# dluvizon/scene-aware-3d-multi-human

Hardware: AMD Instinct MI355X
Metric: optimizer iterations/sec (N humans x T frames) (higher is better)
Workload: dtype f32 (the two dense LBS contractions as split-16-bit MFMA operands -- three products of (hi, lo) fp16 / bf16 terms, fp32 accumulate; everything else plain fp32)

## Files before the change

### include/mhmocap_hip.h

```cpp
#ifndef MHMOCAP_HIP_H
#define MHMOCAP_HIP_H

#include <stddef.h>
#include <stdint.h>

#ifdef __cplusplus
extern "C" {
#endif

#define MH_NUM_JOINTS 24
#define MH_NUM_BETAS 10
#define MH_NUM_POSE_BASIS 207
#define MH_NUM_KP 17
#define MH_FEAT_STRIDE 224

typedef enum mh_status {
  MH_OK = 0,
  MH_ERR_INVALID = -1,
  MH_ERR_HIP = -2,
  MH_ERR_NO_DEVICE = -3,
  MH_ERR_UNSUPPORTED = -4
} mh_status;

typedef struct mh_model mh_model;
// ... 27 lines not shown
};
int mh_profile_enable(int on);
int mh_profile_read(int which, float* ms);
int mh_device_count(void);

int mh_stream_create(void** out_stream);
int mh_stream_destroy(void* stream);
int mh_streams_share_queue(void* stream_a, void* stream_b, float spin_us, int* shared);
int mh_stream_spin(void* stream, float spin_us);

int mh_model_create(mh_model** out, const mh_model_host* host);
int mh_model_destroy(mh_model* m);
const int32_t* mh_model_faces(const mh_model* m);

size_t mh_lbs_workspace_bytes(int B);
int mh_lbs_forward(const mh_model* m, int B, int NB, const float* betas ,
                   const float* poses , const float* xscale ,
                   const float* transl , float* verts ,
                   float* vposed , float* posed_joints ,
                   void* ws, void* stream);

int mh_lbs_forward_ex(const mh_model* m, int B, int NB, const float* betas, const float* poses ,
                      const float* rotmats , const float* xscale, const float* transl, float* verts,
                      float* vposed , float* posed_joints , void* ws, void* stream);
int mh_lbs_forward_rotmats(const mh_model* m, int B, int NB, const float* betas, const float* rotmats ,
                           const float* xscale, const float* transl, float* verts, float* posed_joints ,
                           void* ws, void* stream);

typedef struct mh_fwd_proj {
  float s, w1, h1;
  float ra, rk, thr;
  float slack_ndc, slack_y;
  float thr_soft;
  float* ndc;
  const float* rowb;
  int32_t* bbox;
  int32_t* bbox_prev;
  unsigned long long* lowkey;
  unsigned long long* lowkey_prev;
  int32_t* moved;
  float* clear;
  unsigned long long clear_n;
} mh_fwd_proj;
int mh_lbs_forward_proj(const mh_model* m, int B, int NB, const float* betas, const float* poses,
                        const float* xscale, const float* transl, float* verts, float* vposed ,
                        const mh_fwd_proj* proj, void* ws, void* stream);
int mh_lowest_resolve(const float* verts , int B, int V, unsigned long long* lowkey ,
                      int32_t* low_idx , float* low_xyz , void* stream);

int mh_lbs_set_mode(int split16);
int mh_lbs_get_mode(void);
int mh_lbs_set_forward_pipeline(int on);
int mh_lbs_get_forward_pipeline(void);

int mh_joints_regress(const mh_model* m, int which, int B, const float* verts ,
                      const float* corr , int root_relative_to,
                      float* joints , void* stream);

size_t mh_keypoint_workspace_bytes(const mh_model* m, int B);
int mh_keypoint_terms(const mh_model* m, int B, const float* transl , const float* K_host,
                      const float* Kd_host , const float* joint_w_host ,
                      const float* pose2d , float thr, float img_w, float img_h, float coef,
                      float* kp, float* uv, float* gkp, float* loss, const void* ws, void* ws2 ,
                      void* kp_ws, void* stream);
int mh_lbs_backward_kp(const mh_model* m, int B, int NB, const float* betas, const float* poses,
                       const float* vposed, const float* gverts, float* gposes, float* gtransl,
                       float* gbetas, float* gxscale, void* ws, void* ws2, void* stream);
typedef struct mh_raster_fin mh_raster_fin;
int mh_lbs_backward_kp_fin(const mh_model* m, int B, int NB, const float* betas, const float* poses,
                       const float* vposed, const float* gverts, float* gposes, float* gtransl,
                       float* gbetas, float* gxscale, void* ws, void* ws2, const mh_raster_fin* fin, void* stream);

int mh_lbs_backward_person_partials(const mh_model* m, int B, void* ws2, float** gbeta_b, float** gxs_b);
int mh_lbs_person_reduce(const mh_model* m, int B, int NB, void* ws2, float* gbetas, float* gxscale, void* stream);

size_t mh_lbs_backward_workspace_bytes(int B);
int mh_lbs_backward(const mh_model* m, int B, int NB, const float* betas, const float* poses,
                    const float* xscale, const float* transl, const float* vposed,
                    const float* gverts, const float* gjoints, float* gposes, float* gtransl,
                    float* gbetas, float* gxscale, void* ws, void* ws2, void* stream);
int mh_lbs_backward_ex(const mh_model* m, int B, int NB, const float* betas, const float* poses, const float* rotmats,
                       const float* vposed, const float* gverts, const float* gjoints, const float* gposed,
                       float* gposes, float* grotmats, float* gtransl, float* gbetas, float* gxscale,
                       void* ws, void* ws2, void* stream);
int mh_joints_regress_backward(const mh_model* m, int which, int B, const float* gjoints , int root_relative_to,
                               float* gverts, float* gcorr, void* stream);

int mh_project_joints_loss(int B, const float* joints , const float* K_host,
                           const float* Kd_host, const float* pose2d, float thr, int mode,
                           float img_w, float img_h, float coef, float* uv, float* gjoints,
                           float* loss, void* stream);

int mh_project_joints_loss_w(int B, const float* joints, const float* K_host, const float* Kd_host,
                             const float* joint_w_host, const float* pose2d, float thr, int mode, float img_w,
                             float img_h, float coef, float* uv, float* gjoints, float* loss, void* stream);

int mh_warmup_project(int B, int NB, const float* local_joints , const float* xscale,
                      const float* transl , const float* K_host, const float* Kd_host,
                      const float* pose2d, float thr, float coef, float* gtransl, float* loss,
                      void* stream);

int mh_warmup_project_w(int B, int NB, const float* local_joints, const float* xscale, const float* transl,
                        const float* K_host, const float* Kd_host, const float* joint_w_host, const float* pose2d,
                        float thr, float coef, float* gtransl, float* loss, void* stream);

int mh_rmsprop_step(float* params, const float* grads, float* square_avg, float* momentum_buf,
// ... 224 lines not shown
```

### scene-aware-3d-multi-human_amd/csrc/mh_lbs.hip

```cpp
#include <algorithm>
#include <mutex>
#include <unordered_map>

#include "mh_common.h"
#include "mh_raster_p.h"
#include "mh_experiment.h"

#define MFMA32(a, b, c) __builtin_amdgcn_mfma_f32_32x32x2f32((a), (b), (c), 0, 0, 0)


struct PoseFwdP {
  int B, NB, G;
  const float* betas;
  const float* poses;
  const float* rotmats;
  const float* xscale;
  const float* Jt;
  const float* JS;
  float* featT;
  uint16_t* F16;
  float* A;
  float* scale;
  float* posed;
  mh_tree tree;
  int* bbox;
  int* bbox_prev;
  unsigned long long* lowkey;
  unsigned long long* lowkey_prev;
  int* moved;
  float* clear;
  unsigned long long clear_n;
};

__device__ __forceinline__ void mh_joint_rest(const float* Jt, const float* JS, const float* beta, int j, float J[3]) {
#pragma unroll
  for (int c = 0; c < 3; ++c) {
    float a = Jt[j * 3 + c];
#pragma unroll
    for (int l = 0; l < MH_NUM_BETAS; ++l) a = fmaf(JS[(j * 3 + c) * MH_NUM_BETAS + l], beta[l], a);
    J[c] = a;
  }
}

__device__ __forceinline__ void mh_compose(const float* Gp, const float R[9], const float rel[3], float G[12]) {
#pragma unroll
  for (int r = 0; r < 3; ++r) {
#pragma unroll
    for (int c = 0; c < 3; ++c)
      G[r * 4 + c] = fmaf(Gp[r * 4 + 2], R[6 + c], fmaf(Gp[r * 4 + 1], R[3 + c], Gp[r * 4 + 0] * R[c]));
    G[r * 4 + 3] = fmaf(Gp[r * 4 + 2], rel[2], fmaf(Gp[r * 4 + 1], rel[1], Gp[r * 4 + 0] * rel[0])) + Gp[r * 4 + 3];
  }
}

__global__ __launch_bounds__(256) void k_pose_fwd(PoseFwdP p) {
  __shared__ float sG[8][MH_NJ][12];
  __shared__ float sJ[8][MH_NJ][3];
  if (p.clear)
    for (size_t i = (size_t)blockIdx.x * 256 + threadIdx.x; i < p.clear_n; i += (size_t)gridDim.x * 256) p.clear[i] = 0.f;
  const int bl = threadIdx.x >> 5, j = threadIdx.x & 31;
  const int b = blockIdx.x * 8 + bl;
  const bool valid = b < p.B, act = j < MH_NJ;
  float beta[MH_NUM_BETAS];
#pragma unroll
  for (int l = 0; l < MH_NUM_BETAS; ++l) beta[l] = valid ? p.betas[(size_t)(b % p.NB) * MH_NUM_BETAS + l] : 0.f;
  float R[9] = {1, 0, 0, 0, 1, 0, 0, 0, 1}, J[3] = {0, 0, 0};
  if (valid && act) {
    mh_joint_rest(p.Jt, p.JS, beta, j, J);
    if (p.rotmats) {
#pragma unroll
      for (int e = 0; e < 9; ++e) R[e] = p.rotmats[((size_t)b * MH_NJ + j) * 9 + e];
    } else if (j < 22) {
      float r[3] = {p.poses[(size_t)b * 72 + 3 * j], p.poses[(size_t)b * 72 + 3 * j + 1], p.poses[(size_t)b * 72 + 3 * j + 2]};
      mh_rodrigues(r, R);
    }
    sJ[bl][j][0] = J[0];
    sJ[bl][j][1] = J[1];
    sJ[bl][j][2] = J[2];
  }
  __syncthreads();
  float Gm[12] = {1, 0, 0, 0, 0, 1, 0, 0, 0, 0, 1, 0};
  const int par = act ? p.tree.parent[j] : -1;
  const int lev = act ? p.tree.level[j] : -1;
  float rel[3] = {J[0], J[1], J[2]};
  if (valid && act && j > 0) {
    rel[0] -= sJ[bl][par][0];
    rel[1] -= sJ[bl][par][1];
    rel[2] -= sJ[bl][par][2];
  }
  for (int l = 0; l <= p.tree.maxlevel; ++l) {
    if (valid && act && lev == l) {
      if (l == 0) {
#pragma unroll
        for (int r = 0; r < 3; ++r) {
          Gm[r * 4 + 0] = R[r * 3 + 0];
          Gm[r * 4 + 1] = R[r * 3 + 1];
          Gm[r * 4 + 2] = R[r * 3 + 2];
          Gm[r * 4 + 3] = J[r];
        }
      } else {
        float Gp[12];
#pragma unroll
        for (int e = 0; e < 12; ++e) Gp[e] = sG[bl][par][e];
        mh_compose(Gp, R, rel, Gm);
      }
#pragma unroll
      for (int e = 0; e < 12; ++e) sG[bl][j][e] = Gm[e];
    }
    __syncthreads();
  }
// ... 585 lines not shown
        const float x0 = fmaf(T[2], vp2, fmaf(T[1], vp1, T[0] * vp0)) + T[3];
        const float x1 = fmaf(T[6], vp2, fmaf(T[5], vp1, T[4] * vp0)) + T[7];
        const float x2 = fmaf(T[10], vp2, fmaf(T[9], vp1, T[8] * vp0)) + T[11];
        const f32x3 o = {fmaf(st[0], x0, st[1]), fmaf(st[0], x1, st[2]), fmaf(st[0], x2, st[3])};
        if (FULL || g * 32 + row0 + 4 * lh < p.B) {
          const unsigned off_r = lane_off + (unsigned)row0 * row_b32;
          *(f32x3*)(vg + (size_t)off_r) = o;
          if (qg) {
            const f32x3 q = {vp0, vp1, vp2};
            *(f32x3*)(qg + (size_t)off_r) = q;
          }
          if (PROJ) {
            const float Zc = o[2];
            const float xn = p.P.s * (-o[0]) / Zc + p.P.w1, yn = p.P.s * (-o[1]) / Zc + p.P.h1;
            const f32x3 nd = {xn, yn, Zc};
            *(f32x3*)(ng + (size_t)off_r) = nd;
            const float drow = fabsf(fmaf(-yn, p.P.rk, p.P.ra) - rbv[r]);
            const bool mv = !(drow < p.P.thr_soft);
            const f32x4 th = *(const f32x4*)(sB + 512 + row0 * 16);
            const float ly = *(const float*)(sB + 1024 + row0 * 16);
            const bool zok = Zc > 1e-8f;
            const bool c0 = zok && xn < th[0], c1 = zok && yn < th[1], c2 = zok && xn > th[2], c3 = zok && yn > th[3];
            const bool c4 = o[1] > ly;
            if (__builtin_amdgcn_ballot_w64(c0 || c1 || c2 || c3 || c4 || mv) != 0ull) {
              int b = g * 32 + row0 + 4 * lh;
              asm volatile("" : "+v"(b));
              int* bb = p.P.bbox + (size_t)b * 4;
              if (c0) atomicMin(bb, mh_ord(xn));
              if (c1) atomicMin(bb + 1, mh_ord(yn));
              if (c2) atomicMax(bb + 2, mh_ord(xn));
              if (c3) atomicMax(bb + 3, mh_ord(yn));
              if (c4) atomicMax(p.P.lowkey + b, ((unsigned long long)mh_ordu(o[1] + 0.0f) << 32) | (unsigned)~(unsigned)v_c);
              if (mv) p.P.moved[(drow < p.P.thr ? p.B : 0) + b] = 1;
            }
          }
        }
      }
      __builtin_amdgcn_sched_barrier(0);
    }
    ax = nx; ay = ny; az = nz;
    v_c = v_n; vok_c = vok_n; tv_c = tv_n;
#pragma unroll
    for (int k = 0; k < 4; ++k) { sj_c[k] = sj_n[k]; sw_c[k] = sw_n[k]; }
  }
}

static size_t align256(size_t x) { return (x + 255) & ~(size_t)255; }

struct FwdWs {
  float* featT;
  float* A;
  float* scale;
  uint16_t* F16;
};
static FwdWs carve_fwd(void* ws, int G) {
  char* p = (char*)ws;
  FwdWs w;
  w.featT = (float*)p;
  p += align256((size_t)G * MH_FS * 32 * 4);
  w.A = (float*)p;
  p += align256((size_t)G * 32 * MH_NJ * 12 * 4);
  w.scale = (float*)p;
  p += align256((size_t)G * 32 * 4);
  w.F16 = (uint16_t*)p;
  return w;
}

static std::mutex g_fwd_seen_mu;
static std::unordered_map<const void*, int>& fwd_seen() {
  static std::unordered_map<const void*, int> m;
  return m;
}
static void fwd_note(const void* ws, int B) {
  std::lock_guard<std::mutex> lk(g_fwd_seen_mu);
  fwd_seen()[ws] = B;
}
int mh_lbs_forward_views(int B, const void* ws, const float** featT, const float** A, const float** scale) {
  MH_CHECK(ws && B > 0 && featT && A && scale, "null argument");
  {
    std::lock_guard<std::mutex> lk(g_fwd_seen_mu);
    const auto it = fwd_seen().find(ws);
    MH_CHECK(it != fwd_seen().end() && it->second == B,
             "this workspace does not hold an LBS forward of this many bodies: the key-point term reads the pose features "
             "and bone transforms of the forward that immediately preceded it on the same workspace");
  }
  FwdWs w = carve_fwd(const_cast<void*>(ws), mh_groups(B));
  *featT = w.featT; *A = w.A; *scale = w.scale;
  return MH_OK;
}

static int g_lbs_mode = -1;
static int lbs_mode() {
  if (g_lbs_mode < 0) {
    const char* e = getenv("MHHIP_LBS_FP32");
    g_lbs_mode = (e && e[0] == '1') ? 0 : 1;
  }
  return g_lbs_mode;
}
extern "C" int mh_lbs_set_mode(int split16) {
  g_lbs_mode = split16 ? 1 : 0;
  return MH_OK;
}
extern "C" int mh_lbs_get_mode(void) { return lbs_mode(); }
static int g_fwd_pipe = -1;
static int fwd_pipe() {
  if (g_fwd_pipe < 0) {
    const char* e = getenv("MHHIP_FWD_PIPE");
    g_fwd_pipe = (e && e[0] == '0') ? 0 : 1;
  }
  return g_fwd_pipe;
}
extern "C" int mh_lbs_set_forward_pipeline(int on) {
  MH_CHECK(on == 0 || on == 1, "mh_lbs_set_forward_pipeline: 0 (tile after tile) or 1 (software pipeline)");
  g_fwd_pipe = on;
  return MH_OK;
}
extern "C" int mh_lbs_get_forward_pipeline(void) { return fwd_pipe(); }

extern "C" size_t mh_lbs_workspace_bytes(int B) {
  int G = mh_groups(B < 1 ? 1 : B);
  return align256((size_t)G * MH_FS * 32 * 4) + align256((size_t)G * 32 * MH_NJ * 12 * 4) + align256((size_t)G * 32 * 4) +
         align256((size_t)G * (MH_FS / 16) * 2 * 64 * 16);
}

static int lbs_forward_impl(const mh_model* m, int B, int NB, const float* betas, const float* poses, const float* rotmats,
                            const float* xscale, const float* transl, float* verts, float* vposed, float* posed_joints,
                            void* ws, void* stream, const mh_fwd_proj* proj = nullptr);

extern "C" int mh_lbs_forward_proj(const mh_model* m, int B, int NB, const float* betas, const float* poses,
                                   const float* xscale, const float* transl, float* verts, float* vposed,
                                   const mh_fwd_proj* proj, void* ws, void* stream) {
  MH_CHECK(poses && proj, "null argument");
  MH_CHECK(proj->ndc && proj->rowb && proj->bbox && proj->bbox_prev && proj->lowkey && proj->lowkey_prev && proj->moved,
           "mh_fwd_proj: null target (fill it with mh_raster_forward_targets)");
  MH_CHECK(lbs_mode() != 0, "mh_lbs_forward_proj: the fused epilogue exists for the split-16-bit kernels only (mh_lbs_set_mode(1))");
  return lbs_forward_impl(m, B, NB, betas, poses, nullptr, xscale, transl, verts, vposed, nullptr, ws, stream, proj);
}

extern "C" int mh_lbs_forward(const mh_model* m, int B, int NB, const float* betas, const float* poses,
                              const float* xscale, const float* transl, float* verts, float* vposed,
                              float* posed_joints, void* ws, void* stream) {
  MH_CHECK(poses, "null argument");
  return lbs_forward_impl(m, B, NB, betas, poses, nullptr, xscale, transl, verts, vposed, posed_joints, ws, stream);
}

extern "C" int mh_lbs_forward_rotmats(const mh_model* m, int B, int NB, const float* betas, const float* rotmats,
                                      const float* xscale, const float* transl, float* verts, float* posed_joints,
                                      void* ws, void* stream) {
  MH_CHECK(rotmats, "null argument");
  return lbs_forward_impl(m, B, NB, betas, nullptr, rotmats, xscale, transl, verts, nullptr, posed_joints, ws, stream);
}

extern "C" int mh_lbs_forward_ex(const mh_model* m, int B, int NB, const float* betas, const float* poses, const float* rotmats,
                                 const float* xscale, const float* transl, float* verts, float* vposed, float* posed_joints,
                                 void* ws, void* stream) {
  MH_CHECK((poses != nullptr) != (rotmats != nullptr), "exactly one of poses (axis-angle) and rotmats");
  return lbs_forward_impl(m, B, NB, betas, poses, rotmats, xscale, transl, verts, vposed, posed_joints, ws, stream);
}

static int lbs_forward_impl(const mh_model* m, int B, int NB, const float* betas, const float* poses, const float* rotmats,
                            const float* xscale, const float* transl, float* verts, float* vposed, float* posed_joints,
                            void* ws, void* stream, const mh_fwd_proj* proj) {
  MH_CHECK(m && betas && verts && ws, "null argument");
  MH_CHECK(B > 0 && NB > 0, "B and NB must be positive");
  hipStream_t st = (hipStream_t)stream;
  const int G = mh_groups(B);
  FwdWs w = carve_fwd(ws, G);
  fwd_note(ws, B);
  PoseFwdP pp;
  pp.B = B; pp.NB = NB; pp.G = G;
  pp.betas = betas; pp.poses = poses; pp.rotmats = rotmats; pp.xscale = xscale;
  pp.Jt = m->Jt; pp.JS = m->JS;
  pp.featT = w.featT; pp.A = w.A; pp.scale = w.scale; pp.posed = posed_joints;
  pp.tree = m->tree;
  const bool split16 = lbs_mode() != 0;
  pp.F16 = split16 ? w.F16 : nullptr;
  pp.bbox = proj ? proj->bbox : nullptr; pp.bbox_prev = proj ? proj->bbox_prev : nullptr;
  pp.lowkey = proj ? proj->lowkey : nullptr; pp.lowkey_prev = proj ? proj->lowkey_prev : nullptr;
  pp.moved = proj ? proj->moved : nullptr;
  pp.clear = proj ? proj->clear : nullptr; pp.clear_n = proj ? proj->clear_n : 0ull;
  mh_prof_mark(MH_PROF_POSE_FWD, 0, st);
  hipLaunchKernelGGL(k_pose_fwd, dim3(G * 4), dim3(256), 0, st, pp);
  MH_LAUNCH_CHECK();
  mh_prof_mark(MH_PROF_POSE_FWD, 1, st);
  if (split16) {
    SkinFwd16P sp;
    sp.B = B; sp.G = G; sp.V = m->V; sp.VP = m->VP; sp.nw = m->nw;
    sp.unscale = ldexpf(1.f, -(MH_F16_FEAT_SHIFT + m->d16_shift));
    sp.F16 = w.F16; sp.A = w.A; sp.scale = w.scale; sp.transl = transl;
    sp.D16 = m->D16; sp.vt = m->vt; sp.skidx = m->skidx; sp.skw = m->skw;
    sp.verts = verts; sp.vposed = vposed;
    MH_CHECK((size_t)32 * m->V * 12 < ((size_t)1 << 32), "model too large for 32-bit lane offsets");
#ifdef FWD16_LDS_PAD
    const size_t lds = FWD16_LDS_BYTES + (proj ? 0 : FWD16_LDS_PAD);
#else
    const size_t lds = FWD16_LDS_BYTES;
#endif
    const bool full = (B % 32) == 0, nw4 = m->nw <= 4;
    auto kern = proj ? (full ? (nw4 ? k_skin_fwd16<true, true, true> : k_skin_fwd16<true, false, true>)
                             : (nw4 ? k_skin_fwd16<false, true, true> : k_skin_fwd16<false, false, true>))
                     : (full ? (nw4 ? k_skin_fwd16<true, true, false> : k_skin_fwd16<true, false, false>)
                             : (nw4 ? k_skin_fwd16<false, true, false> : k_skin_fwd16<false, false, false>));
    static unsigned char attr16[8][MH_MAX_DEVICES];
    const int ki = (proj ? 4 : 0) + (full ? 2 : 0) + (nw4 ? 1 : 0);
    sp.P = proj ? *proj : mh_fwd_proj{};
    if (mh_first_on_device(attr16[ki]))
      MH_HIP(hipFuncSetAttribute((const void*)kern, hipFuncAttributeMaxDynamicSharedMemorySize, (int)lds));
    mh_prof_mark(MH_PROF_SKIN_FWD, 0, st);
    const int ntiles = m->VP / 32;
    if (proj && fwd_pipe()) {
      auto kp = full ? (nw4 ? k_skin_fwd16p<true, true, true> : k_skin_fwd16p<true, false, true>)
                     : (nw4 ? k_skin_fwd16p<false, true, true> : k_skin_fwd16p<false, false, true>);
      static unsigned char attrp[4][MH_MAX_DEVICES];
      if (mh_first_on_device(attrp[(full ? 2 : 0) + (nw4 ? 1 : 0)]))
        MH_HIP(hipFuncSetAttribute((const void*)kp, hipFuncAttributeMaxDynamicSharedMemorySize, (int)lds));
      int bpg = std::max(1, 256 / G);
      int tpb = std::min(FWD16_WAVES * 3, (ntiles + bpg - 1) / bpg);
      sp.tpb = tpb;
      bpg = (ntiles + tpb - 1) / tpb;
      hipLaunchKernelGGL(kp, dim3(bpg, G), dim3(FWD16_WAVES * 64), lds, st, sp);
      MH_LAUNCH_CHECK();
      mh_prof_mark(MH_PROF_SKIN_FWD, 1, st);
      return MH_OK;
    }
    int bpg = std::max(1, (2 * 256) / G);
    int tpb = std::min(FWD16_WAVES * FWD16_TPW, (ntiles + bpg - 1) / bpg);
    sp.tpb = tpb;
    bpg = (ntiles + tpb - 1) / tpb;
    hipLaunchKernelGGL(kern, dim3(bpg, G), dim3(FWD16_WAVES * 64), lds, st, sp);
    MH_LAUNCH_CHECK();
    mh_prof_mark(MH_PROF_SKIN_FWD, 1, st);
    return MH_OK;
  }
// ... 287 lines not shown
        for (int r = 0; r < 4; ++r) {
          float* q = sRed + ((14 + t) * 4 + r) * 64 + lane;
          *q = (w == 0) ? accA[t][r] : (*q + accA[t][r]);
        }
      if (lq == 0) {
        float* q = sRed + BWD_NACC * 4 * 64 + li * 4;
        if (w == 0) { q[0] = sT0; q[1] = sT1; q[2] = sT2; q[3] = sS; }
        else { q[0] += sT0; q[1] += sT1; q[2] += sT2; q[3] += sS; }
      }
    }
    __syncthreads();
  }
  const size_t base = (size_t)ch * p.GB + (size_t)g * 16;
  float* oF = p.pF + base * MH_FS;
  for (int i = tid; i < 14 * 4 * 64; i += 256) {
    const int t = i >> 8, r = (i >> 6) & 3, l = i & 63;
    const int row = (l >> 4) * 4 + r;
    oF[(size_t)row * MH_FS + t * 16 + (l & 15)] = sRed[i];
  }
  float* oA = p.pA + base * 288;
  for (int i = tid; i < 24 * 4 * 64; i += 256) {
    const int t = i >> 8, r = (i >> 6) & 3, l = i & 63;
    const int row = (l >> 4) * 4 + r;
    const int joint = (t & 1) * 16 + (l & 15);
    if (joint < MH_NJ) oA[(size_t)row * 288 + (t >> 1) * MH_NJ + joint] = sRed[14 * 256 + i];
  }
  float* oS = p.pS + base * 4;
  for (int i = tid; i < 64; i += 256) oS[i] = sRed[BWD_NACC * 4 * 64 + i];
}

#define MFMA_BF16(a, b, c) __builtin_amdgcn_mfma_f32_32x32x16_bf16((a), (b), (c), 0, 0, 0)
typedef __bf16 bfx8 __attribute__((ext_vector_type(8)));
typedef __bf16 bfx2 __attribute__((ext_vector_type(2)));
typedef float f32x2 __attribute__((ext_vector_type(2)));
typedef float f32x2a __attribute__((ext_vector_type(2), aligned(8)));
typedef unsigned u32x4 __attribute__((ext_vector_type(4)));

__device__ __forceinline__ void mh_split_bf16x8(const float x[8], bfx8& hi, bfx8& lo) {
  u32x4 h, l;
#pragma unroll
  for (int i = 0; i < 4; ++i) {
    const f32x2 v = {x[2 * i], x[2 * i + 1]};
    const unsigned u = __builtin_bit_cast(unsigned, __builtin_convertvector(v, bfx2));
    const f32x2 r = {v[0] - __builtin_bit_cast(float, u << 16), v[1] - __builtin_bit_cast(float, u & 0xffff0000u)};
    h[i] = u;
    l[i] = __builtin_bit_cast(unsigned, __builtin_convertvector(r, bfx2));
  }
  hi = __builtin_bit_cast(bfx8, h);
  lo = __builtin_bit_cast(bfx8, l);
}

struct Bwd16P {
  int B, G, V, VP, nw, CH, PB;
  const float* A;
  const float* scale;
  const float* vposed;
  const float* gverts;
  const float* gjoints;
  const uint16_t* Dt16;
  const uint16_t* W16;
  const int* skidx;
  const float* skw;
  const int* kpv_ptr;
  const int* kpv_j;
  const float* kpv_w;
  const int* kpv_head;
  float* pF;
  float* pA;
  float* pS;
};

#define BW_TS 20
#ifndef SB_OCC
#define SB_OCC 2
#endif
#ifndef SB_FENCE2
#define SB_FENCE2
#endif
#ifndef SB_FENCE
#define SB_FENCE
#endif
#define SB_GS 33
#define SB_LDS_FLOATS (32 * BWD_AS + 32 * 52 + 3 * 16 * SB_GS + 7 * 32 * BW_TS + 3 * 2 * 64 * 4 + 8 * 32 * 3)
template <bool NW4, bool KP>
__global__ __launch_bounds__(256, SB_OCC) void k_skinbwd16(Bwd16P p) {
  extern __shared__ __attribute__((aligned(16))) float smb[];
  float* sA = smb;
  float* sGj = sA + 32 * BWD_AS;
  float* sGv = sGj + 32 * 52;
  float* sGx = sGv + 3 * 16 * SB_GS;
  float* sQ = sGx + 3 * 32 * BW_TS;
  unsigned* sF = (unsigned*)(sQ + 4 * 32 * BW_TS);
  float* sTr = (float*)(sF + 3 * 2 * 64 * 4);
  const int per = gridDim.x >> 3, item = (blockIdx.x & 7) * per + (blockIdx.x >> 3);
  if (item >= p.G * p.CH) return;
  const int g = item % p.G, ch = item / p.G;
  const int tid = threadIdx.x, wave = tid >> 6, lane = tid & 63, li = lane & 31, lh = lane >> 5;
  L_T0();
  for (int i = tid; i < 32 * MH_NJ * 12; i += 256) {
    const int bb = i / (MH_NJ * 12), e = i % (MH_NJ * 12);
    sA[bb * BWD_AS + e] = p.A[(size_t)(g * 32 + bb) * MH_NJ * 12 + e];
  }
  for (int i = tid; i < 32 * 51; i += 256) {
    const int bb = i / 51, e = i % 51;
    const int b = g * 32 + bb;
    sGj[bb * 52 + e] = (p.gjoints && b < p.B) ? p.gjoints[(size_t)b * 51 + e] : 0.f;
  }
  const int bi = tid & 31, vs = tid >> 5;
  const float sb = (g * 32 + bi < p.B) ? p.scale[g * 32 + bi] : 0.f;
  const float* sAb = sA + bi * BWD_AS;
  f32x16 accF[2], accA[3];
#pragma unroll
  for (int i = 0; i < 2; ++i) accF[i] = (f32x16){0};
#pragma unroll
  for (int i = 0; i < 3; ++i) accA[i] = (f32x16){0};
  float sT0 = 0, sT1 = 0, sT2 = 0;
  const int nblk = p.VP / 16;
  const int b0 = ch * p.PB, bend = min((ch + 1) * p.PB, nblk);
  const bool two = wave < 3;
  const int ct0 = 2 * wave, ct1 = two ? 2 * wave + 1 : 6;
  for (int i = tid; i < 32 * BW_TS; i += 256) sQ[3 * 32 * BW_TS + i] = 1.f;
  const bfx8* Db = (const bfx8*)p.Dt16 + lane;
  const bfx8* Wb = (const bfx8*)p.W16 + lane;
  const int fvx = tid & 15, fr = tid >> 4;
  f32x3 rg[2], rq[2];
  auto fetch = [&](int blk) {
    const int v = blk * 16 + fvx;
#pragma unroll
    for (int k = 0; k < 2; ++k) {
      const int b = g * 32 + fr + 16 * k;
      const size_t o = ((size_t)(b < p.B ? b : p.B - 1) * p.V + (v < p.V ? v : p.V - 1)) * 3;
      rq[k] = *(const f32x3*)(p.vposed + o);
      rg[k] = (f32x3){0.f, 0.f, 0.f};
      if (p.gverts) rg[k] = *(const f32x3*)(p.gverts + o);
    }
  };
  int4 j4[2], kh[2];
  f32x4 w4[2];
  auto fetch_rows = [&](int blk) {
    const int vp = blk * 16 + 2 * vs;
#pragma unroll
    for (int u = 0; u < 2; ++u) {
      if (NW4) {
        j4[u] = *(const int4*)(p.skidx + (size_t)(vp + u) * 4);
        w4[u] = *(const f32x4*)(p.skw + (size_t)(vp + u) * 4);
      }
      if (KP) kh[u] = *(const int4*)(p.kpv_head + (size_t)(vp + u) * 4);
    }
  };
  if (b0 < bend) fetch(b0);
  L_MARK(0);
  for (int blk = b0; blk < bend; ++blk) {
    fetch_rows(blk);
#pragma unroll
    for (int k = 0; k < 2; ++k)
#pragma unroll
      for (int c = 0; c < 3; ++c) sGv[(c * 16 + fvx) * SB_GS + fr + 16 * k] = rg[k][c];
    const bfx8* Dk = Db + (size_t)blk * 42 * 64;
    bfx8 bD[3][2][2], bW[2];
    auto fetch_b = [&](int c) {
      bD[c][0][0] = Dk[((c * 7 + ct0) * 2) * 64];
      bD[c][0][1] = Dk[((c * 7 + ct0) * 2 + 1) * 64];
      bD[c][1][0] = Dk[((c * 7 + ct1) * 2) * 64];
      bD[c][1][1] = Dk[((c * 7 + ct1) * 2 + 1) * 64];
    };
    fetch_b(0);
    fetch_b(1);
    fetch_b(2);
    const int vp = blk * 16 + 2 * vs;
    SB_FENCE;
    L_MARK(1);
    __syncthreads();
    L_MARK(2);
#pragma unroll
// ... 59 lines not shown
      gvp[0][u] = fmaf(T[8], gx2, fmaf(T[4], gx1, T[0] * gx0));
      gvp[1][u] = fmaf(T[9], gx2, fmaf(T[5], gx1, T[1] * gx0));
      gvp[2][u] = fmaf(T[10], gx2, fmaf(T[6], gx1, T[2] * gx0));
      __builtin_amdgcn_sched_barrier(0);
    }
    bW[0] = Wb[(size_t)blk * 128];
    bW[1] = Wb[(size_t)blk * 128 + 64];
    {
      const int fl = (vs >> 2) * 32 + bi, fd = vs & 3;
#pragma unroll
      for (int c = 0; c < 3; ++c) {
        const f32x2 v2 = {gvp[c][0], gvp[c][1]};
        const unsigned hi = __builtin_bit_cast(unsigned, __builtin_convertvector(v2, bfx2));
        const f32x2 r2 = {v2[0] - __builtin_bit_cast(float, hi << 16), v2[1] - __builtin_bit_cast(float, hi & 0xffff0000u)};
        sF[((c * 2) * 64 + fl) * 4 + fd] = hi;
        sF[((c * 2 + 1) * 64 + fl) * 4 + fd] = __builtin_bit_cast(unsigned, __builtin_convertvector(r2, bfx2));
        *(f32x2a*)(sGx + (c * 32 + bi) * BW_TS + 2 * vs) = (f32x2a){gxp[c][0], gxp[c][1]};
      }
    }
    L_MARK(3);
    __syncthreads();
    L_MARK(4);
#pragma unroll
    for (int c = 0; c < 3; ++c) {
      const bfx8 ah = *(const bfx8*)(sF + ((c * 2) * 64 + lane) * 4);
      const bfx8 al = *(const bfx8*)(sF + ((c * 2 + 1) * 64 + lane) * 4);
      accF[0] = MFMA_BF16(ah, bD[c][0][0], accF[0]);
      accF[0] = MFMA_BF16(ah, bD[c][0][1], accF[0]);
      accF[0] = MFMA_BF16(al, bD[c][0][0], accF[0]);
      accF[1] = MFMA_BF16(ah, bD[c][1][0], accF[1]);
      accF[1] = MFMA_BF16(ah, bD[c][1][1], accF[1]);
      accF[1] = MFMA_BF16(al, bD[c][1][0], accF[1]);
      SB_FENCE2;
    }
#pragma unroll
    for (int k = 0; k < 3; ++k) {
      const int rc = 3 * wave + k, r = rc >> 2, c = rc & 3;
      const f32x4* gp = (const f32x4*)(sGx + (r * 32 + li) * BW_TS + 8 * lh);
      const f32x4 ga = gp[0], gb = gp[1];
      const f32x4* qp = (const f32x4*)(sQ + (c * 32 + li) * BW_TS + 8 * lh);
      const f32x4 qa = qp[0], qb = qp[1];
      float a[8];
#pragma unroll
      for (int t = 0; t < 4; ++t) { a[t] = ga[t] * qa[t]; a[4 + t] = gb[t] * qb[t]; }
      bfx8 ah, al;
      mh_split_bf16x8(a, ah, al);
      accA[k] = MFMA_BF16(ah, bW[0], accA[k]);
      accA[k] = MFMA_BF16(ah, bW[1], accA[k]);
      accA[k] = MFMA_BF16(al, bW[0], accA[k]);
      SB_FENCE2;
    }
    L_MARK(5);
  }
  const size_t GB = (size_t)p.G * 32;
  const size_t base = (size_t)ch * GB + (size_t)g * 32;
  float* oF = p.pF + base * MH_FS;
  float* oA = p.pA + base * 288;
#pragma unroll
  for (int r = 0; r < 16; ++r) {
    const int row = (r & 3) + 8 * (r >> 2) + 4 * lh;
    oF[(size_t)row * MH_FS + (2 * wave) * 32 + li] = accF[0][r];
    if (two) oF[(size_t)row * MH_FS + (2 * wave + 1) * 32 + li] = accF[1][r];
    if (li < MH_NJ) {
#pragma unroll
      for (int k = 0; k < 3; ++k) oA[(size_t)row * 288 + (3 * wave + k) * MH_NJ + li] = accA[k][r];
    }
  }
  sTr[(vs * 32 + bi) * 3 + 0] = sT0;
  sTr[(vs * 32 + bi) * 3 + 1] = sT1;
  sTr[(vs * 32 + bi) * 3 + 2] = sT2;
  __syncthreads();
  if (tid < 128) {
    const int bb = tid >> 2, c = tid & 3;
    float s = 0.f;
    if (c < 3)
      for (int k = 0; k < 8; ++k) s += sTr[(k * 32 + bb) * 3 + c];
    p.pS[base * 4 + tid] = s;
  }
  L_OUT(8, 6);
}

struct PoseBwdP {
  int B, NB, G, CH;
  const float* betas;
  const float* poses;
  const float* gjoints;
  const float* kp_rowsum;
  const float* rotmats;
  const float* gposed;
  float* grotmats;
  const float* scale;
  const float* A;
  const float* Jt;
  const float* JS;
  const float* pF;
  const float* pA;
  const float* pS;
  float* gposes;
  float* gtransl;
  float* gbeta_b;
  float* gxs_b;
  int scale_from_joint_sums;
  mh_tree tree;
  int has_fin;
  mh_raster_fin fin;
};

__global__ __launch_bounds__(256) void k_pose_bwd(PoseBwdP p) {
  if (p.has_fin && blockIdx.x == 0) {
    __shared__ float f_g0[MH_FIN_U * 256], f_g1[MH_FIN_U * 256];
    mh_raster_finish_job<256>(p.fin, f_g0, f_g1);
    return;
  }
  if (p.has_fin == 2 && blockIdx.x == 1) {
    r_finalize_lists<256>(*(const RasterP*)p.fin.lists);
    return;
  }
  __shared__ float sGA[1][12 * MH_NJ];
  __shared__ float sGF[1][MH_FS];
  __shared__ float sG[1][MH_NJ][12];
  __shared__ float sgG[1][MH_NJ][12];
  __shared__ float sJ[1][MH_NJ][3];
  __shared__ float sgJ[1][MH_NJ][3];
  __shared__ float sS[1][4];
  const size_t GB = (size_t)p.G * 32;
  __shared__ float sP[8][12 * MH_NJ + MH_FS + 4];
  const int g = threadIdx.x >> 5, j = threadIdx.x & 31, bl = 0;
  const int b = (int)blockIdx.x - p.has_fin;
  const bool valid = b < p.B, act = j < MH_NJ;
  float beta[MH_NUM_BETAS];
  float R[9] = {1, 0, 0, 0, 1, 0, 0, 0, 1}, J[3] = {0, 0, 0}, th[3] = {0, 0, 0};
  float Gm[12] = {1, 0, 0, 0, 0, 1, 0, 0, 0, 0, 1, 0};
// ... 167 lines not shown
        for (int k = 0; k < 3; ++k) t += gR[r * 3 + k] * K[cc * 3 + k] + K[k * 3 + r] * gR[k * 3 + cc];
        gK[r * 3 + cc] = s * gR[r * 3 + cc] + omc * t;
      }
    const float gd0 = gK[7] - gK[5], gd1 = gK[2] - gK[6], gd2 = gK[3] - gK[1];
    const float gat = ga - (gd0 * th[0] + gd1 * th[1] + gd2 * th[2]) / (ang * ang);
    float* o = p.gposes + (size_t)b * 72 + 3 * j;
    o[0] += gd0 / ang + gat * a0 / ang;
    o[1] += gd1 / ang + gat * a1 / ang;
    o[2] += gd2 / ang + gat * a2 / ang;
  }
  {
    float a = 0.f;
    if (valid && j < 3 * MH_NUM_BETAS) {
      const int l = j % MH_NUM_BETAS, q0 = (j / MH_NUM_BETAS) * (MH_NJ * 3 / 3);
#pragma unroll 8
      for (int q = q0; q < q0 + MH_NJ * 3 / 3; ++q) a = fmaf(p.JS[q * MH_NUM_BETAS + l], sgJ[bl][q / 3][q % 3], a);
    }
    sP[0][j] = a;
  }
  __syncthreads();
  if (b < p.G * 32 && j < MH_NUM_BETAS)
    p.gbeta_b[(size_t)b * MH_NUM_BETAS + j] = valid ? ((sGF[bl][j] + sP[0][j]) + sP[0][j + MH_NUM_BETAS]) + sP[0][j + 2 * MH_NUM_BETAS] : 0.f;
  if (b < p.G * 32 && j == 31) p.gxs_b[b] = valid ? sS[bl][3] * p.scale[b] * 0.0953101798043249f  : 0.f;
  if (valid && j >= 24 && j < 27 && p.gtransl) {
    const int c = j - 24;
    float a = sS[bl][c];
    if (p.gjoints && p.kp_rowsum)
      for (int q = 0; q < MH_NKP; ++q) a = fmaf(1.f - p.kp_rowsum[q], p.gjoints[((size_t)b * MH_NKP + q) * 3 + c], a);
    p.gtransl[(size_t)b * 3 + c] += a;
  }
}

__global__ __launch_bounds__(256) void k_person_reduce(int B, int NB, const float* gbeta_b, const float* gxs_b,
                                                       float* gbetas, float* gxscale) {
  __shared__ float s[256];
  const int n = blockIdx.x, q = blockIdx.y;
  float a = 0;
  for (int b = n + threadIdx.x * NB; b < B; b += 256 * NB) a += (q < 10) ? gbeta_b[(size_t)b * MH_NUM_BETAS + q] : gxs_b[b];
  s[threadIdx.x] = a;
  __syncthreads();
  for (int o = 128; o > 0; o >>= 1) {
    if (threadIdx.x < o) s[threadIdx.x] += s[threadIdx.x + o];
    __syncthreads();
  }
  if (threadIdx.x == 0) {
    if (q < 10) {
      if (gbetas) gbetas[(size_t)n * MH_NUM_BETAS + q] += s[0];
    } else if (gxscale) {
      gxscale[n] += s[0];
    }
  }
}

static int bwd16_chunks(int G) {
  int ch = (500 + G / 2) / G;
  if (ch < 1) ch = 1;
  if (ch > 54) ch = 54;
  return ch;
}

static int bwd_chunks(int G16) {
  int ch = (512 + G16 / 2) / G16;
  if (ch < 1) ch = 1;
  if (ch > 27) ch = 27;
  return ch;
}

struct BwdWs {
  float* pF;
  float* pA;
  float* pS;
  float* gbeta_b;
  float* gxs_b;
};
static BwdWs carve_bwd(void* ws, int G, int CH) {
  char* p = (char*)ws;
  BwdWs w;
  const size_t GB = (size_t)G * 32;
  w.pF = (float*)p; p += align256((size_t)CH * GB * MH_FS * 4);
  w.pA = (float*)p; p += align256((size_t)CH * GB * 288 * 4);
  w.pS = (float*)p; p += align256((size_t)CH * GB * 4 * 4);
  w.gbeta_b = (float*)p; p += align256(GB * MH_NUM_BETAS * 4);
  w.gxs_b = (float*)p;
  return w;
}

extern "C" size_t mh_lbs_backward_workspace_bytes(int B) {
  const int G = mh_groups(B < 1 ? 1 : B), CH = std::max(bwd_chunks(2 * G), bwd16_chunks(G)) + 1;
  const size_t GB = (size_t)G * 32;
  return align256((size_t)CH * GB * MH_FS * 4) + align256((size_t)CH * GB * 288 * 4) + align256((size_t)CH * GB * 16) +
         align256(GB * MH_NUM_BETAS * 4) + align256(GB * 4);
}

static int lbs_backward_impl(const mh_model* m, int B, int NB, const float* betas, const float* poses, const float* rotmats,
                             const float* vposed, const float* gverts, const float* gjoints, const float* gposed,
                             float* gposes, float* grotmats, float* gtransl, float* gbetas, float* gxscale,
                             void* ws, void* ws2, void* stream, int kp_chunk = 0, const mh_raster_fin* fin = nullptr);

extern "C" int mh_lbs_backward_kp(const mh_model* m, int B, int NB, const float* betas, const float* poses, const float* vposed,
                                  const float* gverts, float* gposes, float* gtransl, float* gbetas, float* gxscale,
                                  void* ws, void* ws2, void* stream) {
  MH_CHECK(poses && gposes, "null argument");
  return lbs_backward_impl(m, B, NB, betas, poses, nullptr, vposed, gverts, nullptr, nullptr, gposes, nullptr, gtransl, gbetas,
                           gxscale, ws, ws2, stream, 1);
}

extern "C" int mh_lbs_backward_kp_fin(const mh_model* m, int B, int NB, const float* betas, const float* poses, const float* vposed,
                                      const float* gverts, float* gposes, float* gtransl, float* gbetas, float* gxscale,
// ... 28 lines not shown

extern "C" int mh_lbs_person_reduce(const mh_model* m, int B, int NB, void* ws2, float* gbetas, float* gxscale, void* stream) {
  float *gb = nullptr, *gx = nullptr;
  const int rc = mh_lbs_backward_person_partials(m, B, ws2, &gb, &gx);
  if (rc != MH_OK) return rc;
  MH_CHECK(NB > 0, "NB must be positive");
  if (!gbetas && !gxscale) return MH_OK;
  hipLaunchKernelGGL(k_person_reduce, dim3(NB, 11), dim3(256), 0, (hipStream_t)stream, B, NB, (const float*)gb, (const float*)gx, gbetas, gxscale);
  MH_LAUNCH_CHECK();
  return MH_OK;
}

extern "C" int mh_lbs_backward(const mh_model* m, int B, int NB, const float* betas, const float* poses,
                               const float* xscale, const float* transl, const float* vposed, const float* gverts,
                               const float* gjoints, float* gposes, float* gtransl, float* gbetas, float* gxscale,
                               void* ws, void* ws2, void* stream) {
  (void)xscale; (void)transl;
  MH_CHECK(poses && gposes, "null argument");
  return lbs_backward_impl(m, B, NB, betas, poses, nullptr, vposed, gverts, gjoints, nullptr, gposes, nullptr, gtransl, gbetas,
                           gxscale, ws, ws2, stream);
}

extern "C" int mh_lbs_backward_ex(const mh_model* m, int B, int NB, const float* betas, const float* poses, const float* rotmats,
                                  const float* vposed, const float* gverts, const float* gjoints, const float* gposed,
                                  float* gposes, float* grotmats, float* gtransl, float* gbetas, float* gxscale,
                                  void* ws, void* ws2, void* stream) {
  MH_CHECK((poses != nullptr) != (rotmats != nullptr), "exactly one of poses (axis-angle) and rotmats");
  MH_CHECK(poses ? gposes != nullptr : grotmats != nullptr, "null gradient output");
  return lbs_backward_impl(m, B, NB, betas, poses, rotmats, vposed, gverts, gjoints, gposed, gposes, grotmats, gtransl, gbetas,
                           gxscale, ws, ws2, stream);
}

static int lbs_backward_impl(const mh_model* m, int B, int NB, const float* betas, const float* poses, const float* rotmats,
                             const float* vposed, const float* gverts, const float* gjoints, const float* gposed,
                             float* gposes, float* grotmats, float* gtransl, float* gbetas, float* gxscale,
                             void* ws, void* ws2, void* stream, int kp_chunk, const mh_raster_fin* fin) {
  MH_CHECK(m && betas && vposed && ws && ws2, "null argument");
  MH_CHECK(gverts || gjoints || kp_chunk, "need gverts and/or gjoints");
  MH_CHECK(B > 0 && NB > 0, "B and NB must be positive");
  MH_CHECK(!gjoints || m->reg[MH_REG_ALPHAPOSE].J == MH_NKP, "gjoints needs the key-point regressor");
  hipStream_t st = (hipStream_t)stream;
  const bool split16 = lbs_mode() != 0;
  const int G = mh_groups(B), G16 = 2 * G, CH = split16 ? bwd16_chunks(G) : bwd_chunks(G16);
  FwdWs fw = carve_fwd(ws, G);
  BwdWs bw = carve_bwd(ws2, G, CH + 1);
  if (split16) {
    Bwd16P sp;
    sp.B = B; sp.G = G; sp.V = m->V; sp.VP = m->VP; sp.nw = m->nw; sp.CH = CH;
    sp.PB = (m->VP / 16 + CH - 1) / CH;
    sp.A = fw.A; sp.scale = fw.scale; sp.vposed = vposed; sp.gverts = gverts; sp.gjoints = gjoints;
    sp.Dt16 = m->Dt16; sp.W16 = m->W16; sp.skidx = m->skidx; sp.skw = m->skw;
    sp.kpv_ptr = m->kpv_ptr; sp.kpv_j = m->kpv_j; sp.kpv_w = m->kpv_w; sp.kpv_head = m->kpv_head;
    sp.pF = bw.pF; sp.pA = bw.pA; sp.pS = bw.pS;
    const size_t ldsB = (size_t)SB_LDS_FLOATS * 4;
    static unsigned char attr_b16[MH_MAX_DEVICES];
    if (mh_first_on_device(attr_b16)) {
      const void* fk[4] = {(const void*)k_skinbwd16<false, false>, (const void*)k_skinbwd16<false, true>,
                           (const void*)k_skinbwd16<true, false>, (const void*)k_skinbwd16<true, true>};
      for (int i = 0; i < 4; ++i) MH_HIP(hipFuncSetAttribute(fk[i], hipFuncAttributeMaxDynamicSharedMemorySize, (int)ldsB));
    }
    const bool nw4 = m->nw == 4, kp = gjoints != nullptr;
    auto kern = nw4 ? (kp ? k_skinbwd16<true, true> : k_skinbwd16<true, false>)
                    : (kp ? k_skinbwd16<false, true> : k_skinbwd16<false, false>);
    mh_prof_mark(MH_PROF_SKIN_BWD, 0, st);
    hipLaunchKernelGGL(kern, dim3(8 * ((G * CH + 7) / 8)), dim3(256), ldsB, st, sp);
    MH_LAUNCH_CHECK();
    mh_prof_mark(MH_PROF_SKIN_BWD, 1, st);
  } else {
  static unsigned char attr_set[MH_MAX_DEVICES];
  const size_t lds = (size_t)(16 * BWD_AS + 16 * 52 + BWD_NACC * 4 * 64 + 64) * 4;
  if (mh_first_on_device(attr_set))
    MH_HIP(hipFuncSetAttribute((const void*)k_skin_bwd, hipFuncAttributeMaxDynamicSharedMemorySize, (int)lds));
  SkinBwdP sp;
  sp.B = B; sp.G16 = G16; sp.GB = G * 32; sp.V = m->V; sp.VP = m->VP; sp.nw = m->nw; sp.CH = CH;
  sp.PQ = (m->VP / 4 + CH - 1) / CH;
  sp.A = fw.A; sp.scale = fw.scale; sp.vposed = vposed; sp.gverts = gverts; sp.gjoints = gjoints;
  sp.Dt = m->Dt; sp.skidx = m->skidx; sp.skw = m->skw;
  sp.kpv_ptr = m->kpv_ptr; sp.kpv_j = m->kpv_j; sp.kpv_w = m->kpv_w;
  sp.pF = bw.pF; sp.pA = bw.pA; sp.pS = bw.pS;
  mh_prof_mark(MH_PROF_SKIN_BWD, 0, st);
  hipLaunchKernelGGL(k_skin_bwd, dim3(G16, CH), dim3(256), lds, st, sp);
  MH_LAUNCH_CHECK();
  mh_prof_mark(MH_PROF_SKIN_BWD, 1, st);
  }
  PoseBwdP pp;
  pp.B = B; pp.NB = NB; pp.G = G; pp.CH = CH + (kp_chunk ? 1 : 0);
  pp.betas = betas; pp.poses = poses; pp.gjoints = gjoints;
  pp.rotmats = rotmats; pp.gposed = gposed; pp.grotmats = grotmats;
  pp.kp_rowsum = m->reg[MH_REG_ALPHAPOSE].rowsum;
  pp.scale = fw.scale; pp.A = fw.A; pp.Jt = m->Jt; pp.JS = m->JS;
  pp.pF = bw.pF; pp.pA = bw.pA; pp.pS = bw.pS;
  pp.gposes = gposes; pp.gtransl = gtransl; pp.gbeta_b = bw.gbeta_b; pp.gxs_b = bw.gxs_b;
  pp.scale_from_joint_sums = split16 ? 1 : 0;
  pp.tree = m->tree;
  pp.has_fin = (fin && fin->B > 0) ? (fin->has_lists ? 2 : 1) : 0;
  if (pp.has_fin) pp.fin = *fin; else memset(&pp.fin, 0, sizeof(pp.fin));
  mh_prof_mark(MH_PROF_POSE_BWD, 0, st);
  hipLaunchKernelGGL(k_pose_bwd, dim3(G * 32 + pp.has_fin), dim3(256), 0, st, pp);
  MH_LAUNCH_CHECK();
  if (gbetas || gxscale) {
    hipLaunchKernelGGL(k_person_reduce, dim3(NB, 11), dim3(256), 0, st, B, NB, bw.gbeta_b, bw.gxs_b, gbetas, gxscale);
    MH_LAUNCH_CHECK();
  }
  mh_prof_mark(MH_PROF_POSE_BWD, 1, st);
  return MH_OK;
}
```

Before: 1550.

## Make split-16 skinning backward a persistent kernel with atomic work claiming

The split-16 LBS backward kernel now launches a fixed number of workgroups (occupancy times CU count by default) that loop, claiming items from eight per-XCD atomic counters and stealing from other buckets once their own is empty. Per-item setup such as the sQ ones-fill is hoisted out of the loop, and the A and gjoints staging into LDS now uses 128-bit vector loads. The counters are zeroed in the pose-forward kernel, and the last workgroup to finish resets them. The aim is to cut tail imbalance and launch cost, at the price of atomics, an extra barrier per item and a dependence on the forward kernel having reset the counters.

```diff
diff --git a/include/mhmocap_hip.h b/include/mhmocap_hip.h
--- a/include/mhmocap_hip.h
+++ b/include/mhmocap_hip.h
@@ -103,6 +103,10 @@
 int mh_lbs_get_mode(void);
 int mh_lbs_set_forward_pipeline(int on);
 int mh_lbs_get_forward_pipeline(void);
+int mh_lbs_set_backward_workgroups(int n);
+int mh_lbs_get_backward_workgroups(void);
+int mh_lbs_set_backward_items(int items);
+int mh_lbs_get_backward_items(void);
 
 int mh_joints_regress(const mh_model* m, int which, int B, const float* verts ,
                       const float* corr , int root_relative_to,
diff --git a/scene-aware-3d-multi-human_amd/csrc/mh_lbs.hip b/scene-aware-3d-multi-human_amd/csrc/mh_lbs.hip
--- a/scene-aware-3d-multi-human_amd/csrc/mh_lbs.hip
+++ b/scene-aware-3d-multi-human_amd/csrc/mh_lbs.hip
@@ -9,6 +9,7 @@
 #define MFMA32(a, b, c) __builtin_amdgcn_mfma_f32_32x32x2f32((a), (b), (c), 0, 0, 0)
 
 
+#define MH_BWD_CLAIM_INTS 16
 struct PoseFwdP {
   int B, NB, G;
   const float* betas;
@@ -30,6 +31,7 @@
   int* moved;
   float* clear;
   unsigned long long clear_n;
+  int* claim;
 };
 
 __device__ __forceinline__ void mh_joint_rest(const float* Jt, const float* JS, const float* beta, int j, float J[3]) {
@@ -55,6 +57,7 @@
 __global__ __launch_bounds__(256) void k_pose_fwd(PoseFwdP p) {
   __shared__ float sG[8][MH_NJ][12];
   __shared__ float sJ[8][MH_NJ][3];
+  if (blockIdx.x == 0 && threadIdx.x < MH_BWD_CLAIM_INTS) p.claim[threadIdx.x] = 0;
   if (p.clear)
     for (size_t i = (size_t)blockIdx.x * 256 + threadIdx.x; i < p.clear_n; i += (size_t)gridDim.x * 256) p.clear[i] = 0.f;
   const int bl = threadIdx.x >> 5, j = threadIdx.x & 31;
@@ -746,6 +749,7 @@
   float* A;
   float* scale;
   uint16_t* F16;
+  int* claim;
 };
 static FwdWs carve_fwd(void* ws, int G) {
   char* p = (char*)ws;
@@ -757,6 +761,8 @@
   w.scale = (float*)p;
   p += align256((size_t)G * 32 * 4);
   w.F16 = (uint16_t*)p;
+  p += align256((size_t)G * (MH_FS / 16) * 2 * 64 * 16);
+  w.claim = (int*)p;
   return w;
 }
 
@@ -814,7 +820,7 @@
 extern "C" size_t mh_lbs_workspace_bytes(int B) {
   int G = mh_groups(B < 1 ? 1 : B);
   return align256((size_t)G * MH_FS * 32 * 4) + align256((size_t)G * 32 * MH_NJ * 12 * 4) + align256((size_t)G * 32 * 4) +
-         align256((size_t)G * (MH_FS / 16) * 2 * 64 * 16);
+         align256((size_t)G * (MH_FS / 16) * 2 * 64 * 16) + align256(MH_BWD_CLAIM_INTS * 4);
 }
 
 static int lbs_forward_impl(const mh_model* m, int B, int NB, const float* betas, const float* poses, const float* rotmats,
@@ -873,6 +879,7 @@
   pp.lowkey = proj ? proj->lowkey : nullptr; pp.lowkey_prev = proj ? proj->lowkey_prev : nullptr;
   pp.moved = proj ? proj->moved : nullptr;
   pp.clear = proj ? proj->clear : nullptr; pp.clear_n = proj ? proj->clear_n : 0ull;
+  pp.claim = w.claim;
   mh_prof_mark(MH_PROF_POSE_FWD, 0, st);
   hipLaunchKernelGGL(k_pose_fwd, dim3(G * 4), dim3(256), 0, st, pp);
   MH_LAUNCH_CHECK();
@@ -1266,6 +1273,8 @@
 
 struct Bwd16P {
   int B, G, V, VP, nw, CH, PB;
+  int per;
+  int* claim;
   const float* A;
   const float* scale;
   const float* vposed;
@@ -1306,21 +1315,61 @@
   float* sQ = sGx + 3 * 32 * BW_TS;
   unsigned* sF = (unsigned*)(sQ + 4 * 32 * BW_TS);
   float* sTr = (float*)(sF + 3 * 2 * 64 * 4);
-  const int per = gridDim.x >> 3, item = (blockIdx.x & 7) * per + (blockIdx.x >> 3);
-  if (item >= p.G * p.CH) return;
+  __shared__ int sItem;
+  const int tid = threadIdx.x, wave = tid >> 6, lane = tid & 63, li = lane & 31, lh = lane >> 5;
+  const int nitems = p.G * p.CH;
+  int steal = 0, nxt = -1;
+  auto claim = [&]() -> int {
+    while (steal < 8) {
+      const int x = (blockIdx.x + steal) & 7;
+      const int cnt = min(p.per, nitems - x * p.per);
+      if (cnt > 0) {
+        const int pos = atomicAdd(p.claim + x, 1);
+        if (pos < cnt) return x * p.per + pos;
+      }
+      ++steal;
+    }
+    return -1;
+  };
+  if (tid == 0) nxt = claim();
+  const int bi = tid & 31, vs = tid >> 5;
+  const bool two = wave < 3;
+  const int ct0 = 2 * wave, ct1 = two ? 2 * wave + 1 : 6;
+  for (int i = tid; i < 32 * BW_TS; i += 256) sQ[3 * 32 * BW_TS + i] = 1.f;
+  for (;;) {
+  if (tid == 0) sItem = nxt;
+  __syncthreads();
+  const int item = sItem;
+  if (item < 0) break;
   const int g = item % p.G, ch = item / p.G;
-  const int tid = threadIdx.x, wave = tid >> 6, lane = tid & 63, li = lane & 31, lh = lane >> 5;
   L_T0();
-  for (int i = tid; i < 32 * MH_NJ * 12; i += 256) {
-    const int bb = i / (MH_NJ * 12), e = i % (MH_NJ * 12);
-    sA[bb * BWD_AS + e] = p.A[(size_t)(g * 32 + bb) * MH_NJ * 12 + e];
-  }
-  for (int i = tid; i < 32 * 51; i += 256) {
-    const int bb = i / 51, e = i % 51;
-    const int b = g * 32 + bb;
-    sGj[bb * 52 + e] = (p.gjoints && b < p.B) ? p.gjoints[(size_t)b * 51 + e] : 0.f;
-  }
-  const int bi = tid & 31, vs = tid >> 5;
+  {
+    int tp = tid;
+    asm volatile("" : "+v"(tp));
+    const f32x4* A4 = (const f32x4*)(p.A + (size_t)g * 32 * MH_NJ * 12);
+    for (int i = tp; i < 32 * (MH_NJ * 3); i += 256) {
+      const int bb = i / (MH_NJ * 3), q = i % (MH_NJ * 3);
+      *(f32x4*)(sA + bb * BWD_AS + 4 * q) = A4[i];
+    }
+    const int nv = p.gjoints ? max(0, min(32, p.B - g * 32)) * 51 : 0;
+    const float* gj = p.gjoints ? p.gjoints + (size_t)g * 32 * 51 : nullptr;
+    if (nv && (((size_t)gj & 15) == 0)) {
+      for (int i = tp; i < 32 * 51 / 4; i += 256) {
+        f32x4 v = (f32x4){0.f, 0.f, 0.f, 0.f};
+        if (4 * i + 3 < nv) v = *(const f32x4*)(gj + 4 * i);
+        else
+          for (int k = 0; k < 4; ++k)
+            if (4 * i + k < nv) v[k] = gj[4 * i + k];
+#pragma unroll
+        for (int k = 0; k < 4; ++k) {
+          const int e = 4 * i + k;
+          sGj[(e / 51) * 52 + e % 51] = v[k];
+        }
+      }
+    } else {
+      for (int i = tp; i < 32 * 51; i += 256) sGj[(i / 51) * 52 + i % 51] = i < nv ? gj[i] : 0.f;
+    }
+  }
   const float sb = (g * 32 + bi < p.B) ? p.scale[g * 32 + bi] : 0.f;
   const float* sAb = sA + bi * BWD_AS;
   f32x16 accF[2], accA[3];
@@ -1331,9 +1380,6 @@
   float sT0 = 0, sT1 = 0, sT2 = 0;
   const int nblk = p.VP / 16;
   const int b0 = ch * p.PB, bend = min((ch + 1) * p.PB, nblk);
-  const bool two = wave < 3;
-  const int ct0 = 2 * wave, ct1 = two ? 2 * wave + 1 : 6;
-  for (int i = tid; i < 32 * BW_TS; i += 256) sQ[3 * 32 * BW_TS + i] = 1.f;
   const bfx8* Db = (const bfx8*)p.Dt16 + lane;
   const bfx8* Wb = (const bfx8*)p.W16 + lane;
   const int fvx = tid & 15, fr = tid >> 4;
@@ -1499,32 +1545,39 @@
     }
     L_MARK(5);
   }
+  if (tid == 0) nxt = claim();
+  int te = tid;
+  asm volatile("" : "+v"(te));
+  const int ew = te >> 6, eli = te & 31, elh = (te >> 5) & 1;
   const size_t GB = (size_t)p.G * 32;
   const size_t base = (size_t)ch * GB + (size_t)g * 32;
   float* oF = p.pF + base * MH_FS;
   float* oA = p.pA + base * 288;
 #pragma unroll
   for (int r = 0; r < 16; ++r) {
-    const int row = (r & 3) + 8 * (r >> 2) + 4 * lh;
-    oF[(size_t)row * MH_FS + (2 * wave) * 32 + li] = accF[0][r];
-    if (two) oF[(size_t)row * MH_FS + (2 * wave + 1) * 32 + li] = accF[1][r];
-    if (li < MH_NJ) {
-#pragma unroll
-      for (int k = 0; k < 3; ++k) oA[(size_t)row * 288 + (3 * wave + k) * MH_NJ + li] = accA[k][r];
-    }
-  }
-  sTr[(vs * 32 + bi) * 3 + 0] = sT0;
-  sTr[(vs * 32 + bi) * 3 + 1] = sT1;
-  sTr[(vs * 32 + bi) * 3 + 2] = sT2;
+    const int row = (r & 3) + 8 * (r >> 2) + 4 * elh;
+    oF[(size_t)row * MH_FS + (2 * ew) * 32 + eli] = accF[0][r];
+    if (ew < 3) oF[(size_t)row * MH_FS + (2 * ew + 1) * 32 + eli] = accF[1][r];
+    if (eli < MH_NJ) {
+#pragma unroll
+      for (int k = 0; k < 3; ++k) oA[(size_t)row * 288 + (3 * ew + k) * MH_NJ + eli] = accA[k][r];
+    }
+  }
+  sTr[te * 3 + 0] = sT0;
+  sTr[te * 3 + 1] = sT1;
+  sTr[te * 3 + 2] = sT2;
   __syncthreads();
-  if (tid < 128) {
-    const int bb = tid >> 2, c = tid & 3;
+  if (te < 128) {
+    const int bb = te >> 2, c = te & 3;
     float s = 0.f;
     if (c < 3)
       for (int k = 0; k < 8; ++k) s += sTr[(k * 32 + bb) * 3 + c];
-    p.pS[base * 4 + tid] = s;
+    p.pS[base * 4 + te] = s;
   }
   L_OUT(8, 6);
+  }
+  if (tid == 0 && atomicAdd(p.claim + 8, 1) == (int)gridDim.x - 1)
+    for (int x = 0; x < 9; ++x) atomicExch(p.claim + x, 0);
 }
 
 struct PoseBwdP {
@@ -1798,8 +1851,52 @@
   }
 }
 
+#define MH_BWD_ITEMS_DEFAULT 500
+static int g_bwd_items = -1;
+static int bwd_items() {
+  if (g_bwd_items < 0) {
+    const char* e = getenv("MHHIP_BWD_ITEMS");
+    const int v = e ? atoi(e) : 0;
+    g_bwd_items = (v >= 1 && v <= 4000) ? v : MH_BWD_ITEMS_DEFAULT;
+  }
+  return g_bwd_items;
+}
+extern "C" int mh_lbs_set_backward_items(int items) {
+  MH_CHECK(items == 0 || (items >= 1 && items <= 4000), "mh_lbs_set_backward_items: 1..4000, or 0 for the default");
+  g_bwd_items = items ? items : MH_BWD_ITEMS_DEFAULT;
+  return MH_OK;
+}
+extern "C" int mh_lbs_get_backward_items(void) { return bwd_items(); }
+static int g_bwd_wgs = -1;
+static int bwd_wgs() {
+  if (g_bwd_wgs < 0) {
+    const char* e = getenv("MHHIP_BWD_WORKGROUPS");
+    const int v = e ? atoi(e) : 0;
+    g_bwd_wgs = (v >= 1 && v <= 65536) ? v : 0;
+  }
+  return g_bwd_wgs;
+}
+extern "C" int mh_lbs_set_backward_workgroups(int n) {
+  MH_CHECK(n >= 0 && n <= 65536, "mh_lbs_set_backward_workgroups: 0 (two per compute unit) .. 65536");
+  g_bwd_wgs = n;
+  return MH_OK;
+}
+extern "C" int mh_lbs_get_backward_workgroups(void) { return bwd_wgs(); }
+static int mh_cu_count(int* out) {
+  static int cus[MH_MAX_DEVICES];
+  int d = 0, n = 0;
+  MH_HIP(hipGetDevice(&d));
+  const bool slot = d >= 0 && d < MH_MAX_DEVICES;
+  if (slot && cus[d]) { *out = cus[d]; return MH_OK; }
+  MH_HIP(hipDeviceGetAttribute(&n, hipDeviceAttributeMultiprocessorCount, d));
+  MH_CHECK(n > 0, "the device reports no compute units");
+  if (slot) cus[d] = n;
+  *out = n;
+  return MH_OK;
+}
+
 static int bwd16_chunks(int G) {
-  int ch = (500 + G / 2) / G;
+  int ch = (bwd_items() + G / 2) / G;
   if (ch < 1) ch = 1;
   if (ch > 54) ch = 54;
   return ch;
@@ -1934,6 +2031,10 @@
     sp.Dt16 = m->Dt16; sp.W16 = m->W16; sp.skidx = m->skidx; sp.skw = m->skw;
     sp.kpv_ptr = m->kpv_ptr; sp.kpv_j = m->kpv_j; sp.kpv_w = m->kpv_w; sp.kpv_head = m->kpv_head;
     sp.pF = bw.pF; sp.pA = bw.pA; sp.pS = bw.pS;
+    sp.per = (G * CH + 7) / 8; sp.claim = fw.claim;
+    int ncu = 0;
+    if (int rc = mh_cu_count(&ncu)) return rc;
+    const int nwg = std::min(bwd_wgs() ? bwd_wgs() : SB_OCC * ncu, G * CH);
     const size_t ldsB = (size_t)SB_LDS_FLOATS * 4;
     static unsigned char attr_b16[MH_MAX_DEVICES];
     if (mh_first_on_device(attr_b16)) {
@@ -1945,7 +2046,7 @@
     auto kern = nw4 ? (kp ? k_skinbwd16<true, true> : k_skinbwd16<true, false>)
                     : (kp ? k_skinbwd16<false, true> : k_skinbwd16<false, false>);
     mh_prof_mark(MH_PROF_SKIN_BWD, 0, st);
-    hipLaunchKernelGGL(kern, dim3(8 * ((G * CH + 7) / 8)), dim3(256), ldsB, st, sp);
+    hipLaunchKernelGGL(kern, dim3(nwg), dim3(256), ldsB, st, sp);
     MH_LAUNCH_CHECK();
     mh_prof_mark(MH_PROF_SKIN_BWD, 1, st);
   } else {
```

Result: slower. 1482 (-4.4%).
